# thomaspingel/neilpy

Measured on AMD Instinct MI355X. Metric: Mcells/s through SMRF progressive_filter, 16384x16384 fp32 DEM, higher is better.
Workload: dtype f32

## Files before the change

neilpy_amd/csrc/ero_inc_adopt.inc:

```
inline constexpr unsigned char kEroIncAdoptF32[65] = {
    0, 0, 0, 0, 0, 0, 0, 0, 0, 0, 0, 0, 0, 0, 0, 0, 0,
    0, 0, 0, 0, 1, 0, 0, 0, 0, 0, 0, 1, 1, 0, 1, 0, 0,
    1, 0, 1, 0, 1, 0, 1, 1, 1, 1, 0, 1, 1, 1, 1, 1, 1,
    0, 0, 0, 0, 0, 0, 0, 0, 0, 0, 0, 0, 0, 0};
```

neilpy_amd/csrc/morph_incero.h:

```cpp
#pragma once
#include "morph_ring.h"

namespace smrf {

#include "ero_inc.inc"
#include "ero_inc_adopt.inc"

#define SMRF_INCERO_MIN_RADIUS 16
#define SMRF_INCERO_MAX_RADIUS 64

template <typename T>
struct IncEroArgs {
  const T* e_prev;
  const T* last;
  T* out;
  int rows, cols;
  long long ld;
  int seg;
  int nt;
  int plain_tiles;
};

template <int R>
struct IncEroCfg {
  static constexpr int N = kEroInc[R].n;
  static constexpr int DY = kEroInc[R].reach;
  static constexpr int TW = 256, NP = 4, ROWS = 2 * NP;
  static constexpr int W = TW + 2 * DY;
  static constexpr int NPOS = (W + TW - 1) / TW;
  static constexpr int NACC = 2 * DY + ROWS;
  static constexpr int G = 4;
  static constexpr int NJ = NP * N;
  static constexpr int NG = (NJ + G - 1) / G;
  static constexpr int gsize(int g) { const int n = NJ - g * G; return n < 0 ? 0 : n > G ? G : n; }
  static constexpr int dy(int k) { return kEroInc[R].p[k].dy; }
  static constexpr int dx(int k) { return kEroInc[R].p[k].dx; }
  static constexpr int DELTA = (ROWS - (2 * DY) % ROWS) % ROWS;
  static constexpr int LDS_CELLS = N > 0 ? 2 * NP * W : 1;
};

template <typename T, int R>
__global__ __launch_bounds__(256) void inc_erode_kernel(const IncEroArgs<T> a) {
  using C = IncEroCfg<R>;
  using T2 = typename Vec2<T>::type;
  constexpr int N = C::N, DY = C::DY, TW = C::TW, NP = C::NP, ROWS = C::ROWS, W = C::W, NPOS = C::NPOS, NACC = C::NACC, G = C::G;
  __shared__ T2 L[C::LDS_CELLS];
  const int tid = threadIdx.x;
  int bx, by;
  smrf_xcd_tile(a.plain_tiles, [] { return true; }, bx, by);
  const int x0 = bx * TW, x = x0 + tid;
  const int ys = by * a.seg, ye = min(a.rows, ys + a.seg);
  if (ys >= ye) return;
  const int xc = x < a.cols ? x : a.cols - 1;
  const int xl = smrf_fold(xc - 1, a.cols), xr = smrf_fold(xc + 1, a.cols);
  int cpos[NPOS];
  bool act[NPOS];
#pragma unroll
  for (int i = 0; i < NPOS; ++i) {
    act[i] = tid + i * TW < W;
    cpos[i] = smrf_fold(x0 - DY + tid + (act[i] ? i * TW : 0), a.cols);
  }
  T acc[NACC];
#pragma unroll
  for (int i = 0; i < NACC; ++i) acc[i] = ident<T>(false);

  int o0 = ys - 2 * DY - C::DELTA;
  const int nb = (ye - o0 + ROWS - 1) / ROWS;
  RowFold rf(o0 + DY, a.rows);
  T2 pf[NP][NPOS];
  auto prefetch = [&]() {
#pragma unroll
    for (int p = 0; p < NP; ++p) {
      const T* ra = a.last + (long long)rf.at(2 * p) * a.ld;
      const T* rb = a.last + (long long)rf.at(2 * p + 1) * a.ld;
#pragma unroll
      for (int i = 0; i < NPOS; ++i)
        if (i < NPOS - 1 || act[i]) { pf[p][i].x = ra[cpos[i]]; pf[p][i].y = rb[cpos[i]]; }
    }
    rf.advance(ROWS);
  };
  if constexpr (N > 0) prefetch();

  for (int b = 0; b < nb; ++b, o0 += ROWS) {
    const unsigned lds_b = (unsigned)(size_t)(__attribute__((address_space(3))) void*)(L + (b & 1) * NP * W + tid);
    if constexpr (N > 0) {
#pragma unroll
      for (int p = 0; p < NP; ++p)
#pragma unroll
        for (int i = 0; i < NPOS; ++i)
          if (i < NPOS - 1 || act[i]) lds_write2(lds_b + (unsigned)((p * W + i * TW) * (int)sizeof(T2)), pf[p][i]);
      lds_wait<0>();
      __syncthreads();
      if (b + 1 < nb) prefetch();
    }
    const bool store = o0 >= ys;
    T ec[ROWS + 2], el[ROWS], er[ROWS];
    if (store) {
      RowFold rfe(o0 - 1, a.rows);
#pragma unroll
      for (int j = 0; j < ROWS + 2; ++j) {
        const T* row = a.e_prev + (long long)rfe.at(j) * a.ld;
        ec[j] = row[xc];
        if (j >= 1 && j <= ROWS) { el[j - 1] = row[xl]; er[j - 1] = row[xr]; }
      }
    }
    if constexpr (N > 0) {
      T2 rd[2 * G][2];
      auto issue = [&]<int J>(std::integral_constant<int, J>) {
        constexpr int p = J / N, k = J % N;
        constexpr int offl = (p * W + DY - C::dx(k)) * (int)sizeof(T2), offr = (p * W + DY + C::dx(k)) * (int)sizeof(T2);
        rd[J % (2 * G)][0] = lds_read2<offl>(lds_b, T());
        rd[J % (2 * G)][1] = lds_read2<offr>(lds_b, T());
      };
      auto apply = [&]<int J>(std::integral_constant<int, J>) {
        constexpr int p = J / N, k = J % N, s = 2 * p - C::dy(k) + DY;
        static_assert(s >= 0 && s + 1 < NACC, "slot outside the ring");
        op3_acc<false>(acc[s], rd[J % (2 * G)][0].x, rd[J % (2 * G)][1].x);
        op3_acc<false>(acc[s + 1], rd[J % (2 * G)][0].y, rd[J % (2 * G)][1].y);
      };
      auto issue_group = [&]<int Gi>(std::integral_constant<int, Gi>) {
        [&]<int... I>(std::integer_sequence<int, I...>) {
          (issue(std::integral_constant<int, Gi * G + I>{}), ...);
        }(std::make_integer_sequence<int, C::gsize(Gi)>{});
      };
      auto apply_group = [&]<int Gi>(std::integral_constant<int, Gi>) {
        [&]<int... I>(std::integer_sequence<int, I...>) {
          (apply(std::integral_constant<int, Gi * G + I>{}), ...);
        }(std::make_integer_sequence<int, C::gsize(Gi)>{});
      };
      issue_group(std::integral_constant<int, 0>{});
      [&]<int... Gi>(std::integer_sequence<int, Gi...>) {
        (([&] {
           if constexpr (Gi + 1 < C::NG) {
             issue_group(std::integral_constant<int, Gi + 1>{});
             lds_wait<2 * C::gsize(Gi + 1)>();
           } else {
             lds_wait<0>();
           }
           apply_group(std::integral_constant<int, Gi>{});
         }()),
         ...);
      }(std::make_integer_sequence<int, C::NG>{});
    }
    if (store) {
#pragma unroll
      for (int j = 0; j < ROWS; ++j) {
        T m = op3<false>(ec[j + 1], el[j], er[j]);
        m = op3<false>(m, ec[j], ec[j + 2]);
        if constexpr (N > 0) m = op2<false>(m, acc[j]);
        const int o = o0 + j;
        if (o < ye && x < a.cols) smrf_store_out(a.out + (long long)o * a.ld + x, m, a.nt);
      }
    }
    if constexpr (N > 0) {
#pragma unroll
      for (int s = 0; s < NACC - ROWS; ++s) acc[s] = acc[s + ROWS];
#pragma unroll
      for (int s = NACC - ROWS; s < NACC; ++s) acc[s] = ident<T>(false);
    }
  }
}

template <typename T, int R>
int inc_erode_launch(const IncEroArgs<T>& a_in, hipStream_t stream) {
  using C = IncEroCfg<R>;
  constexpr auto kern = inc_erode_kernel<T, R>;
  int resident;
  bool first;
  if (int rc = smrf_resident<kern>(C::TW, 0, resident, first)) return rc;
  if (first && smrf_sw().ring_debug)
    fprintf(stderr, "smrf inc erode: R=%d pairs=%d reach=%d LDS=%zu, %d workgroups/CU resident\n", R, C::N, C::DY,
            C::LDS_CELLS * 2 * sizeof(T), resident);
  IncEroArgs<T> a = a_in;
  const int strips = (a.cols + C::TW - 1) / C::TW;
  a.seg = smrf_seg_len(a.rows, strips, resident, smrf_sw().ring_rounds, 2 * C::DY + C::DELTA, C::ROWS, std::max(32, 4 * C::DY),
                       smrf_sw().seg_rule, a.seg);
  a.plain_tiles = smrf_sw().xcd_remap ? 0 : 1;
  dim3 grid(strips, (a.rows + a.seg - 1) / a.seg);
  hipLaunchKernelGGL(kern, grid, dim3(C::TW), 0, stream, a);
  SMRF_LAUNCH_CHECK();
  return SMRF_OK;
}

}
```

Baseline: 4231.

## Reorder incremental-erode LDS reads by slot and defer output stores one batch

The incremental erosion kernel now applies its LDS neighbour reads in a compile-time plan sorted by accumulator slot. The first write to each slot folds in the shifted value from the previous batch, which removes the per-batch ring shift and identity reset. The global prefetch moves after the e_prev loads inside scheduling barriers, and each batch's output stores are deferred to the next iteration so they overlap with later work. Inactive lanes now do unconditional loads and LDS writes, using a redirected offset, and the per-radius adoption table changes for two radii. The cost is higher register pressure from the old[] copy and the held output values.

```diff
diff --git a/neilpy_amd/csrc/ero_inc_adopt.inc b/neilpy_amd/csrc/ero_inc_adopt.inc
--- a/neilpy_amd/csrc/ero_inc_adopt.inc
+++ b/neilpy_amd/csrc/ero_inc_adopt.inc
@@ -1,5 +1,5 @@
 inline constexpr unsigned char kEroIncAdoptF32[65] = {
     0, 0, 0, 0, 0, 0, 0, 0, 0, 0, 0, 0, 0, 0, 0, 0, 0,
     0, 0, 0, 0, 1, 0, 0, 0, 0, 0, 0, 1, 1, 0, 1, 0, 0,
-    1, 0, 1, 0, 1, 0, 1, 1, 1, 1, 0, 1, 1, 1, 1, 1, 1,
+    0, 0, 1, 0, 1, 0, 1, 1, 1, 1, 1, 1, 1, 1, 1, 1, 1,
     0, 0, 0, 0, 0, 0, 0, 0, 0, 0, 0, 0, 0, 0};
diff --git a/neilpy_amd/csrc/morph_incero.h b/neilpy_amd/csrc/morph_incero.h
--- a/neilpy_amd/csrc/morph_incero.h
+++ b/neilpy_amd/csrc/morph_incero.h
@@ -35,6 +35,35 @@
   static constexpr int gsize(int g) { const int n = NJ - g * G; return n < 0 ? 0 : n > G ? G : n; }
   static constexpr int dy(int k) { return kEroInc[R].p[k].dy; }
   static constexpr int dx(int k) { return kEroInc[R].p[k].dx; }
+  static constexpr int slot(int j) { return 2 * (j / N) - dy(j % N) + DY; }
+  struct Plan { short seq[NJ > 0 ? NJ : 1], first[NACC]; };
+  static constexpr Plan make_plan() {
+    Plan pl{};
+    int n = 0;
+    for (int s = 0; s < NACC; ++s) {
+      pl.first[s] = NJ;
+      for (int j = 0; j < NJ; ++j)
+        if (slot(j) == s) pl.seq[n++] = (short)j;
+    }
+    for (int i = NJ - 1; i >= 0; --i) pl.first[slot(pl.seq[i])] = pl.first[slot(pl.seq[i]) + 1] = (short)i;
+    return pl;
+  }
+  static constexpr Plan plan = make_plan();
+  static constexpr bool plan_ok() {
+    int seen[NJ > 0 ? NJ : 1] = {};
+    for (int i = 0; i < NJ; ++i) ++seen[plan.seq[i]];
+    for (int j = 0; j < NJ; ++j)
+      if (seen[j] != 1) return false;
+    for (int s = 0; s < NACC; ++s) {
+      int firsts = 0, touches = 0;
+      for (int i = 0; i < NJ; ++i)
+        for (int h = 0; h < 2; ++h)
+          if (slot(plan.seq[i]) + h == s) { ++touches; firsts += plan.first[s] == i; }
+      if (firsts != (touches > 0)) return false;
+      if (s + ROWS < NACC && plan.first[s] < NJ && plan.first[s + ROWS] < NJ && plan.first[s] >= plan.first[s + ROWS]) return false;
+    }
+    return true;
+  }
   static constexpr int DELTA = (ROWS - (2 * DY) % ROWS) % ROWS;
   static constexpr int LDS_CELLS = N > 0 ? 2 * NP * W : 1;
 };
@@ -64,6 +93,7 @@
 #pragma unroll
   for (int i = 0; i < NACC; ++i) acc[i] = ident<T>(false);
 
+  static_assert(C::plan_ok(), "the batch plan");
   int o0 = ys - 2 * DY - C::DELTA;
   const int nb = (ye - o0 + ROWS - 1) / ROWS;
   RowFold rf(o0 + DY, a.rows);
@@ -75,12 +105,18 @@
       const T* rb = a.last + (long long)rf.at(2 * p + 1) * a.ld;
 #pragma unroll
       for (int i = 0; i < NPOS; ++i)
-        if (i < NPOS - 1 || act[i]) { pf[p][i].x = ra[cpos[i]]; pf[p][i].y = rb[cpos[i]]; }
+        { pf[p][i].x = ra[cpos[i]]; pf[p][i].y = rb[cpos[i]]; }
     }
     rf.advance(ROWS);
   };
   if constexpr (N > 0) prefetch();
 
+  T outv[ROWS];
+  auto store_rows = [&](int ob) {
+#pragma unroll
+    for (int j = 0; j < ROWS; ++j)
+      if (ob + j < ye && x < a.cols) smrf_store_out(a.out + (long long)(ob + j) * a.ld + x, outv[j], a.nt);
+  };
   for (int b = 0; b < nb; ++b, o0 += ROWS) {
     const unsigned lds_b = (unsigned)(size_t)(__attribute__((address_space(3))) void*)(L + (b & 1) * NP * W + tid);
     if constexpr (N > 0) {
@@ -88,11 +124,11 @@
       for (int p = 0; p < NP; ++p)
 #pragma unroll
         for (int i = 0; i < NPOS; ++i)
-          if (i < NPOS - 1 || act[i]) lds_write2(lds_b + (unsigned)((p * W + i * TW) * (int)sizeof(T2)), pf[p][i]);
+          lds_write2(lds_b + (unsigned)((p * W + (i < NPOS - 1 || act[i] ? i * TW : 0)) * (int)sizeof(T2)), pf[p][i]);
       lds_wait<0>();
       __syncthreads();
-      if (b + 1 < nb) prefetch();
-    }
+    }
+    if (o0 - ROWS >= ys) store_rows(o0 - ROWS);
     const bool store = o0 >= ys;
     T ec[ROWS + 2], el[ROWS], er[ROWS];
     if (store) {
@@ -105,18 +141,35 @@
       }
     }
     if constexpr (N > 0) {
+      __builtin_amdgcn_sched_barrier(0);
+      prefetch();
+      __builtin_amdgcn_sched_barrier(0);
+      T old[NACC];
+#pragma unroll
+      for (int s = 0; s < NACC; ++s) old[s] = acc[s];
+      [&]<int... S>(std::integer_sequence<int, S...>) {
+        (([&] {
+           if constexpr (C::plan.first[S] == C::NJ) acc[S] = S + ROWS < NACC ? old[S + ROWS] : ident<T>(false);
+         }()),
+         ...);
+      }(std::make_integer_sequence<int, NACC>{});
       T2 rd[2 * G][2];
-      auto issue = [&]<int J>(std::integral_constant<int, J>) {
-        constexpr int p = J / N, k = J % N;
+      auto issue = [&]<int I>(std::integral_constant<int, I>) {
+        constexpr int J = C::plan.seq[I], p = J / N, k = J % N;
         constexpr int offl = (p * W + DY - C::dx(k)) * (int)sizeof(T2), offr = (p * W + DY + C::dx(k)) * (int)sizeof(T2);
-        rd[J % (2 * G)][0] = lds_read2<offl>(lds_b, T());
-        rd[J % (2 * G)][1] = lds_read2<offr>(lds_b, T());
-      };
-      auto apply = [&]<int J>(std::integral_constant<int, J>) {
-        constexpr int p = J / N, k = J % N, s = 2 * p - C::dy(k) + DY;
-        static_assert(s >= 0 && s + 1 < NACC, "slot outside the ring");
-        op3_acc<false>(acc[s], rd[J % (2 * G)][0].x, rd[J % (2 * G)][1].x);
-        op3_acc<false>(acc[s + 1], rd[J % (2 * G)][0].y, rd[J % (2 * G)][1].y);
+        rd[I % (2 * G)][0] = lds_read2<offl>(lds_b, T());
+        rd[I % (2 * G)][1] = lds_read2<offr>(lds_b, T());
+      };
+      auto update = [&]<int S, int I>(std::integral_constant<int, S>, std::integral_constant<int, I>, const T& l, const T& r) {
+        static_assert(S >= 0 && S < NACC, "slot outside the ring");
+        if constexpr (C::plan.first[S] != I) op3_acc<false>(acc[S], l, r);
+        else if constexpr (S + ROWS < NACC) acc[S] = op3<false>(old[S + ROWS], l, r);
+        else acc[S] = op2<false>(l, r);
+      };
+      auto apply = [&]<int I>(std::integral_constant<int, I> i) {
+        constexpr int s = C::slot(C::plan.seq[I]);
+        update(std::integral_constant<int, s>{}, i, rd[I % (2 * G)][0].x, rd[I % (2 * G)][1].x);
+        update(std::integral_constant<int, s + 1>{}, i, rd[I % (2 * G)][0].y, rd[I % (2 * G)][1].y);
       };
       auto issue_group = [&]<int Gi>(std::integral_constant<int, Gi>) {
         [&]<int... I>(std::integer_sequence<int, I...>) {
@@ -148,17 +201,11 @@
         T m = op3<false>(ec[j + 1], el[j], er[j]);
         m = op3<false>(m, ec[j], ec[j + 2]);
         if constexpr (N > 0) m = op2<false>(m, acc[j]);
-        const int o = o0 + j;
-        if (o < ye && x < a.cols) smrf_store_out(a.out + (long long)o * a.ld + x, m, a.nt);
+        outv[j] = m;
       }
     }
-    if constexpr (N > 0) {
-#pragma unroll
-      for (int s = 0; s < NACC - ROWS; ++s) acc[s] = acc[s + ROWS];
-#pragma unroll
-      for (int s = NACC - ROWS; s < NACC; ++s) acc[s] = ident<T>(false);
-    }
-  }
+  }
+  if (o0 - ROWS >= ys) store_rows(o0 - ROWS);
 }
 
 template <typename T, int R>
```

Result: faster. 4319, median of 6 (+2.1%).
